# arpitbansal297/Cold-Diffusion-Models

Measured on NVIDIA H100. Metric: training-step images/sec (CelebA-128 deblur UNet, config 3), higher is better.
Workload: dtype tf32

## Files before the change

### cold_diffusion_models_b200/csrc/wgrad_tc.cu

```cuda
#include "tc_common.cuh"

namespace {

constexpr int kMmaWarps = 8;
constexpr int kThreads = 32 * (kMmaWarps + 1);
constexpr int kMaxTaps = 8;
constexpr int kMaxGroups = 4;
constexpr int kMaxAccCols = 256;

struct WgParams {
  int B, Hg, Wg;
  int CW, R, KR;
  int chunks_x, chunks_y, total_chunks, chunks_per_split, splits;
  int Cout, Cin;
  int tiles_co, tiles_ci;
  int ngroups;
  int ntaps[kMaxGroups];
  int nloads[kMaxGroups];
  int tap_index[kMaxGroups][kMaxTaps];
  int tap_load[kMaxGroups][kMaxTaps];
  int tap_shift[kMaxGroups][kMaxTaps];
  int load_dy[kMaxGroups][kMaxTaps], load_dx[kMaxGroups][kMaxTaps];
  int halo;
  int sy, sx;
  int oys, oxs, oy0, ox0;
  int per_batch, chunks_per_img, splits_per_img;
  long long dw_batch_stride;
  float* dw;
  float* db;
};

__device__ __forceinline__ float lds_sw(const uint8_t* base, int row, int c) {
  return cd_round_tf32(*reinterpret_cast<const float*>(base + row * 128 + ((((c >> 2) ^ row) & 7) << 4) + (c & 3) * 4));
}
__device__ __forceinline__ void mma_tf32_16x8x8(float (&d)[4], const float (&a)[4], const float (&b)[2]) {
  asm volatile("mma.sync.aligned.m16n8k8.row.col.f32.tf32.tf32.f32 {%0, %1, %2, %3}, {%4, %5, %6, %7}, {%8, %9}, {%0, %1, %2, %3};"
               : "+f"(d[0]), "+f"(d[1]), "+f"(d[2]), "+f"(d[3])
               : "r"(__float_as_uint(a[0])), "r"(__float_as_uint(a[1])), "r"(__float_as_uint(a[2])), "r"(__float_as_uint(a[3])),
                 "r"(__float_as_uint(b[0])), "r"(__float_as_uint(b[1])));
}
__device__ __forceinline__ void red_add_v2(float* addr, float a, float b) {
  asm volatile("red.global.add.v2.f32 [%0], {%1, %2};" :: "l"(addr), "f"(a), "f"(b) : "memory");
}

template <int BN, int NT, bool BIAS>
__global__ void __launch_bounds__(kThreads, 1)
wgrad_tc_kernel(const __grid_constant__ CUtensorMap mapDY, const __grid_constant__ CUtensorMap mapX,
                const WgParams p, int stages, int a_bytes, int b_bytes, int b_tx_bytes) {
  constexpr int NCH = BN / 32;
  constexpr int NJ = BN / 16;
  static_assert(NT * BN <= kMaxAccCols, "accumulators of one CTA");
  extern __shared__ uint8_t smem_raw[];
  const uint32_t raw_addr = smem_u32(smem_raw);
  uint8_t* smem = smem_raw + ((1024u - (raw_addr & 1023u)) & 1023u);
  const int g = blockIdx.z;
  const int nl = p.nloads[g];
  const int stage_bytes = a_bytes + nl * b_bytes;
  uint64_t* bars = reinterpret_cast<uint64_t*>(smem + stages * stage_bytes);
  uint64_t* full_bar = bars;
  uint64_t* empty_bar = bars + stages;
  const int warp = threadIdx.x >> 5, lane = threadIdx.x & 31;

  if (threadIdx.x == 0) {
    for (int i = 0; i < stages; ++i) { mbar_init(&full_bar[i], 1); mbar_init(&empty_bar[i], kMmaWarps); }
    asm volatile("fence.mbarrier_init.release.cluster;" ::: "memory");
  }
  __syncthreads();

  const int tile = blockIdx.x;
  const int co0 = (tile % p.tiles_co) * 128, ci0 = (tile / p.tiles_co) * BN;
  const int split = blockIdx.y;
  int c_beg = split * p.chunks_per_split;
  int c_end = c_beg + p.chunks_per_split; if (c_end > p.total_chunks) c_end = p.total_chunks;
  long long dw_off = 0;
  if (p.per_batch) {
    const int n = split / p.splits_per_img, sp = split % p.splits_per_img;
    c_beg = n * p.chunks_per_img + sp * p.chunks_per_split;
    c_end = c_beg + p.chunks_per_split;
    if (c_end > (n + 1) * p.chunks_per_img) c_end = (n + 1) * p.chunks_per_img;
    dw_off = n * p.dw_batch_stride;
  }
  const int nchunks = c_end > c_beg ? c_end - c_beg : 0;
// ... 63 lines not shown
#pragma unroll
      for (int t = 0; t < NT; ++t) {
        const uint8_t* sBt = sB + tap_load[t] * b_bytes;
#pragma unroll
        for (int j = 0; j < NJ; ++j) {
          const int cl = wn * (BN / 2) + j * 8 + gq;
          const uint8_t* sBc = sBt + (cl >> 5) * (b_bytes / NCH);
          const float b[2] = {lds_sw(sBc, r0 + tap_shift[t], cl & 31), lds_sw(sBc, r1 + tap_shift[t], cl & 31)};
          mma_tf32_16x8x8(acc[t][0][j], a[0], b);
          mma_tf32_16x8x8(acc[t][1][j], a[1], b);
        }
      }
    }
    __syncwarp();
    if (lane == 0) mbar_arrive(&empty_bar[stage]);
  }
  if (nchunks == 0) return;
#pragma unroll
  for (int t = 0; t < NT; ++t) {
    if (t >= p.ntaps[g]) break;
#pragma unroll
    for (int i = 0; i < 2; ++i) {
#pragma unroll
      for (int h = 0; h < 2; ++h) {
        const int co = co0 + wm * 32 + i * 16 + gq + h * 8;
        if (co >= p.Cout) continue;
        float* wrow = p.dw + dw_off + (static_cast<long long>(p.tap_index[g][t]) * p.Cout + co) * p.Cin;
#pragma unroll
        for (int j = 0; j < NJ; ++j) {
          const int ci = ci0 + wn * (BN / 2) + j * 8 + tq * 2;
          if (ci < p.Cin) red_add_v2(wrow + ci, acc[t][i][j][2 * h], acc[t][i][j][2 * h + 1]);
        }
      }
    }
  }
  if (BIAS && bias_cta) {
#pragma unroll
    for (int i = 0; i < 2; ++i)
#pragma unroll
      for (int h = 0; h < 2; ++h) {
        float v = bsum[i][h];
        v += __shfl_xor_sync(0xffffffffu, v, 1);
        v += __shfl_xor_sync(0xffffffffu, v, 2);
        const int co = co0 + wm * 32 + i * 16 + gq + h * 8;
        if (tq == 0 && co < p.Cout) atomicAdd(p.db + co, v);
      }
  }
}

constexpr int kWmThreads = 512;
constexpr int kWmKR = 64;
constexpr int kWmRegsLow = 40, kWmRegsHigh = 216;

template <int CW> struct WmGeom {
  static constexpr int R = kWmKR / CW, RL = CW + 8;
  static constexpr int kXBox = RL * (R + 2) * 128;
  static constexpr int kXBytes = 2 * kXBox;
  static_assert(kXBox % 1024 == 0, "X boxes keep 1024-byte alignment");
};
template <int BN> struct WmTiles {
  static constexpr int kRawBox = kWmKR * 128;
  static constexpr int kRawBytes = (BN / 32) * kRawBox;
  static constexpr int kBBytes = BN * kWmKR * 4;
};

template <int BN, int NTW, int CW>
__device__ __forceinline__ void wm_consume(const WgParams& p, const uint8_t* smem, int stages, int stage_bytes, uint64_t* afull,
                                           uint64_t* aempty, uint64_t* bfull, uint64_t* bempty, int nchunks, int g, int tbeg,
                                           int co0, int ci0) {
  using G = WmGeom<CW>;
  using T = WmTiles<BN>;
  const int lane = threadIdx.x & 31, w = (threadIdx.x & 127) >> 5, gq = lane >> 2, tq = lane & 3;
  int off[NTW][4];
  const int c = 16 * (w & 1) + gq;
#pragma unroll
  for (int t = 0; t < NTW; ++t) {
#pragma unroll
    for (int h = 0; h < 2; ++h) {
      const int row = p.tap_shift[g][tbeg + t] + 2 * tq + h;
      const int o = (w >> 1) * G::kXBox + row * 128 + ((((c >> 2) ^ row) & 7) << 4) + (c & 3) * 4;
      off[t][2 * h] = o;
      off[t][2 * h + 1] = o ^ 32;
    }
  }
  float acc[NTW][BN / 2];
  uint32_t fr[2][NTW][4];
  auto load_frags = [&](uint32_t (&f)[NTW][4], const uint8_t* xs, int ks) {
    const int kofs = (((ks * 8) / CW) * G::RL + (ks * 8) % CW) * 128;
#pragma unroll
    for (int t = 0; t < NTW; ++t)
#pragma unroll
      for (int e = 0; e < 4; ++e) f[t][e] = __float_as_uint(cd_round_tf32(*reinterpret_cast<const float*>(xs + off[t][e] + kofs)));
  };
  if (nchunks == 0) return;
  mbar_wait(&afull[0], 0);
  load_frags(fr[0], smem, 0);
  for (int it = 0; it < nchunks; ++it) {
    const uint32_t s = it % stages, ph = (it / stages) & 1u;
    mbar_wait(&bfull[s], ph);
    const uint8_t* xs = smem + s * stage_bytes;
    const uint32_t bs = smem_u32(xs + G::kXBytes + T::kRawBytes);
#pragma unroll
    for (int ks = 0; ks < kWmKR / 8; ++ks) {
      wgmma_fence();
      const uint64_t db = make_kmajor_sw128_desc(bs + (ks >> 2) * (BN * 128)) + uint64_t((ks & 3) * 2);
#pragma unroll
      for (int t = 0; t < NTW; ++t) wgmma_tf32_rs<BN>(acc[t], fr[ks & 1][t], db, (it | ks) != 0 ? 1u : 0u);
      wgmma_commit();
      if (ks + 1 < kWmKR / 8) {
        load_frags(fr[(ks + 1) & 1], xs, ks + 1);
      } else if (it + 1 < nchunks) {
        const uint32_t s1 = (it + 1) % stages, ph1 = ((it + 1) / stages) & 1u;
        mbar_wait(&afull[s1], ph1);
        load_frags(fr[0], smem + s1 * stage_bytes, 0);
      }
      wgmma_wait<0>();
    }
    __syncwarp();
    if (lane == 0) { mbar_arrive(&aempty[s]); mbar_arrive(&bempty[s]); }
  }
#pragma unroll
  for (int t = 0; t < NTW; ++t) {
    float* wt = p.dw + static_cast<long long>(p.tap_index[g][tbeg + t]) * p.Cout * p.Cin + ci0 + 16 * w + gq;
#pragma unroll
    for (int j = 0; j < BN / 8; ++j)
#pragma unroll
      for (int e = 0; e < 4; ++e) {
        const int co = co0 + 8 * j + 2 * tq + (e & 1);
        if (co < p.Cout) atomicAdd(wt + static_cast<long long>(co) * p.Cin + (e >> 1) * 8, acc[t][4 * j + e]);
      }
  }
}

template <int BN, int NT, int CW>
__global__ void __launch_bounds__(kWmThreads, 1)
wgrad_wgmma_kernel(const __grid_constant__ CUtensorMap mapDY, const __grid_constant__ CUtensorMap mapX, const __grid_constant__ WgParams p,
                   int stages) {
  using G = WmGeom<CW>;
  using T = WmTiles<BN>;
  constexpr int kStage = G::kXBytes + T::kRawBytes + T::kBBytes;
  extern __shared__ uint8_t smem_raw[];
  const uint32_t raw_addr = smem_u32(smem_raw);
  uint8_t* smem = smem_raw + ((1024u - (raw_addr & 1023u)) & 1023u);
  uint64_t* bars = reinterpret_cast<uint64_t*>(smem + stages * kStage);
  uint64_t* afull = bars;
  uint64_t* aempty = bars + stages;
  uint64_t* rfull = bars + 2 * stages;
  uint64_t* rempty = bars + 3 * stages;
  uint64_t* bfull = bars + 4 * stages;
  uint64_t* bempty = bars + 5 * stages;
  const int warp = threadIdx.x >> 5, lane = threadIdx.x & 31, wg = threadIdx.x >> 7;
  const int g = blockIdx.z, nt = p.ntaps[g];
  const int ncons = nt > NT ? 2 : 1;
  if (threadIdx.x == 0) {
    for (int i = 0; i < stages; ++i) {
      mbar_init(&afull[i], 1); mbar_init(&aempty[i], 4 * ncons);
      mbar_init(&rfull[i], 1); mbar_init(&rempty[i], 4);
      mbar_init(&bfull[i], 4); mbar_init(&bempty[i], 4 * ncons);
    }
    asm volatile("fence.mbarrier_init.release.cluster;" ::: "memory");
  }
  __syncthreads();

  const int tile = blockIdx.x;
  const int co0 = (tile % p.tiles_co) * BN, ci0 = (tile / p.tiles_co) * 64;
  const int c_beg = blockIdx.y * p.chunks_per_split;
  int c_end = c_beg + p.chunks_per_split; if (c_end > p.total_chunks) c_end = p.total_chunks;
  const int nchunks = c_end > c_beg ? c_end - c_beg : 0;

  if (wg == 0) {
    asm volatile("setmaxnreg.dec.sync.aligned.u32 %0;" :: "n"(kWmRegsLow));
    if (warp != 0) return;
    for (int it = 0; it < nchunks; ++it) {
      const int ch = c_beg + it;
      const int gx0 = (ch % p.chunks_x) * CW, gy0 = ((ch / p.chunks_x) % p.chunks_y) * G::R, n = ch / (p.chunks_x * p.chunks_y);
      const uint32_t s = it % stages, ph = (it / stages) & 1u;
      const uint32_t sx = smem_u32(smem + s * kStage);
      mbar_wait(&rempty[s], ph ^ 1u);
      if (elect_one()) {
        mbar_expect_tx(&rfull[s], T::kRawBytes);
#pragma unroll
        for (int b = 0; b < BN / 32; ++b)
          tma_load_4d(sx + G::kXBytes + b * T::kRawBox, &mapDY, &rfull[s], co0 + 32 * b, gx0, gy0, n);
      }
      __syncwarp();
      mbar_wait(&aempty[s], ph ^ 1u);
      if (elect_one()) {
        mbar_expect_tx(&afull[s], G::kXBytes);
        tma_load_4d(sx, &mapX, &afull[s], ci0, gx0 - 1, gy0 - 1, n);
        tma_load_4d(sx + G::kXBox, &mapX, &afull[s], ci0 + 32, gx0 - 1, gy0 - 1, n);
      }
      __syncwarp();
    }
    return;
  }
  if (wg == 1) {
    asm volatile("setmaxnreg.dec.sync.aligned.u32 %0;" :: "n"(kWmRegsLow));
    const int w4 = warp & 3;
    for (int it = 0; it < nchunks; ++it) {
      const uint32_t s = it % stages, ph = (it / stages) & 1u;
      mbar_wait(&rfull[s], ph);
      mbar_wait(&bempty[s], ph ^ 1u);
      const uint8_t* raw = smem + s * kStage + G::kXBytes;
      uint8_t* bt = smem + s * kStage + G::kXBytes + T::kRawBytes;
#pragma unroll 4
      for (int u = w4; u < (BN / 32) * (kWmKR / 4); u += 4) {
        const int b = u % (BN / 32), kq = u / (BN / 32);
        const int co = 32 * b + lane;
        const uint8_t* src = raw + b * T::kRawBox + (lane & 3) * 4;
        float v[4];
#pragma unroll
        for (int j = 0; j < 4; ++j) {
          const int px = 8 * (kq >> 1) + (kq & 1) + 2 * j;
          v[j] = cd_round_tf32(*reinterpret_cast<const float*>(src + px * 128 + ((((lane >> 2) ^ px) & 7) << 4)));
        }
        *reinterpret_cast<float4*>(bt + (kq >> 3) * (BN * 128) + co * 128 + (((kq ^ co) & 7) << 4)) = make_float4(v[0], v[1], v[2], v[3]);
      }
      asm volatile("fence.proxy.async.shared::cta;" ::: "memory");
      __syncwarp();
      if (lane == 0) { mbar_arrive(&rempty[s]); mbar_arrive(&bfull[s]); }
    }
    return;
  }
  const int tbeg = (wg - 2) * NT;
  const int ntw = nt - tbeg < NT ? nt - tbeg : NT;
  if (ntw <= 0) return;
  asm volatile("setmaxnreg.inc.sync.aligned.u32 %0;" :: "n"(kWmRegsHigh));
  if constexpr (NT == 4) {
    if (ntw == 4) wm_consume<BN, 4, CW>(p, smem, stages, kStage, afull, aempty, bfull, bempty, nchunks, g, tbeg, co0, ci0);
    else if (ntw == 3) wm_consume<BN, 3, CW>(p, smem, stages, kStage, afull, aempty, bfull, bempty, nchunks, g, tbeg, co0, ci0);
    else if (ntw == 2) wm_consume<BN, 2, CW>(p, smem, stages, kStage, afull, aempty, bfull, bempty, nchunks, g, tbeg, co0, ci0);
    else wm_consume<BN, 1, CW>(p, smem, stages, kStage, afull, aempty, bfull, bempty, nchunks, g, tbeg, co0, ci0);
  } else {
    if (ntw == 2) wm_consume<BN, 2, CW>(p, smem, stages, kStage, afull, aempty, bfull, bempty, nchunks, g, tbeg, co0, ci0);
    else wm_consume<BN, 1, CW>(p, smem, stages, kStage, afull, aempty, bfull, bempty, nchunks, g, tbeg, co0, ci0);
  }
}

int g_wg_mode = 1;
int g_sms = 0;

template <int BN, int NT>
int launch_wg(bool bias, dim3 grid, size_t smem, cudaStream_t st, const CUtensorMap& mapDY, const CUtensorMap& mapX,
              const WgParams& p, int stages, int a_bytes, int b_bytes, int b_tx) {
  if (bias) {
    CD_CUDA(cudaFuncSetAttribute(wgrad_tc_kernel<BN, NT, true>, cudaFuncAttributeMaxDynamicSharedMemorySize, (int)smem));
    wgrad_tc_kernel<BN, NT, true><<<grid, kThreads, smem, st>>>(mapDY, mapX, p, stages, a_bytes, b_bytes, b_tx);
  } else {
    CD_CUDA(cudaFuncSetAttribute(wgrad_tc_kernel<BN, NT, false>, cudaFuncAttributeMaxDynamicSharedMemorySize, (int)smem));
    wgrad_tc_kernel<BN, NT, false><<<grid, kThreads, smem, st>>>(mapDY, mapX, p, stages, a_bytes, b_bytes, b_tx);
  }
  CD_LAUNCH_CHECK();
  return 0;
}

}

extern "C" int cd_wgrad_tc_set_mode(int mode) { g_wg_mode = mode; return 0; }

static int g_wg_bias_fusion = 0;
extern "C" int cd_wgrad_tc_set_bias_fusion(int enable) { g_wg_bias_fusion = enable; return 0; }

static int g_split_policy = 3;
static int g_split_over_clk = 12000;
extern "C" int cd_wgrad_tc_set_split(int policy, int over_clk) { g_split_policy = policy; if (over_clk > 0) g_split_over_clk = over_clk; return 0; }

static int choose_splits(int tg, int total_chunks, int max_splits, int sms, double chunk_clk) {
  if (max_splits < 1) max_splits = 1;
  int s;
  if (g_split_policy == 0) s = cd_cdiv(2 * sms, tg);
  else if (g_split_policy == 1) s = sms / tg;
  else if (g_split_policy == 2) s = 2 * sms / tg;
  else {
    double best = 1e30; s = 1;
    for (int c = 1; c <= max_splits && c * tg <= 4 * sms + tg; ++c) {
      const int cps = cd_cdiv(total_chunks, c);
      const int real = cd_cdiv(total_chunks, cps);
      const double cost = double(cd_cdiv(static_cast<long long>(tg) * real, sms)) * (cps * chunk_clk + g_split_over_clk);
      if (cost < best) { best = cost; s = c; }
    }
  }
  if (s > max_splits) s = max_splits;
  if (s < 1) s = 1;
  return s;
}

template <int BN, int NT, int CW>
static int launch_wm(dim3 grid, cudaStream_t st, const CUtensorMap& mapDY, const CUtensorMap& mapX, const WgParams& p) {
  constexpr int kStage = WmGeom<CW>::kXBytes + WmTiles<BN>::kRawBytes + WmTiles<BN>::kBBytes;
  int stages = (224 * 1024) / kStage; if (stages > 5) stages = 5;
  static_assert((224 * 1024) / kStage >= 2, "two stages of the wgmma weight-gradient kernel fit shared memory");
  const size_t smem = size_t(stages) * kStage + 1024 + 256;
  auto kern = wgrad_wgmma_kernel<BN, NT, CW>;
  static bool attr_done = false;
  if (!attr_done) {
    CD_CUDA(cudaFuncSetAttribute(kern, cudaFuncAttributeMaxDynamicSharedMemorySize, (int)smem));
    attr_done = true;
  }
  kern<<<grid, kWmThreads, smem, st>>>(mapDY, mapX, p, stages);
  CD_LAUNCH_CHECK();
  return 0;
}

static int wgrad_wgmma(const CdConvDesc* d, const float* dout, int dout_ld, float* dw, EncodeTiledFn enc, cudaStream_t st) {
  const CdConvSrc& c = d->s[0];
  if (c.w_per_batch || d->sy != 1 || d->sx != 1 || d->oys != 1 || d->oxs != 1 || d->oy0 != 0 || d->ox0 != 0) return 1;
  if (c.H != d->Hg || c.W != d->Wg || d->Ho != d->Hg || d->Wo != d->Wg) return 1;
  if (c.C % 64 != 0 || d->Cout % 64 != 0 || c.ntaps < 2 || c.ntaps > 9) return 1;
  for (int t = 0; t < c.ntaps; ++t) if (c.dy[t] < -1 || c.dy[t] > 1 || c.dx[t] < -1 || c.dx[t] > 1) return 1;
  const int CW = d->Wg >= 16 ? 16 : 8, R = kWmKR / CW;
  if (d->Hg < R) return 1;
  const int BN = d->Cout % 128 == 0 ? 128 : 64;
  const int NT = BN == 128 ? 2 : 4;
  WgParams p{};
  p.B = d->B; p.Hg = d->Hg; p.Wg = d->Wg; p.Cout = d->Cout; p.Cin = c.C;
  p.sy = 1; p.sx = 1; p.oys = 1; p.oxs = 1;
  p.dw = dw;
  p.CW = CW; p.R = R; p.KR = kWmKR;
  p.ngroups = cd_cdiv(c.ntaps, 2 * NT);
  for (int gk = 0; gk < p.ngroups; ++gk) {
    const int t0 = gk * 2 * NT, n = c.ntaps - t0 < 2 * NT ? c.ntaps - t0 : 2 * NT;
    p.ntaps[gk] = n;
    for (int k = 0; k < n; ++k) {
      p.tap_index[gk][k] = t0 + k;
      p.tap_shift[gk][k] = (c.dy[t0 + k] + 1) * (CW + 8) + c.dx[t0 + k] + 1;
    }
  }
  p.chunks_x = d->Wg / CW; p.chunks_y = d->Hg / R;
  p.total_chunks = d->B * p.chunks_x * p.chunks_y;
  p.tiles_co = d->Cout / BN; p.tiles_ci = c.C / 64;
  const int tiles = p.tiles_co * p.tiles_ci;
  const int max_taps = p.ntaps[0];
  const double chunk_clk = double(max_taps) * (kWmKR / 8) * (BN / 2);
  const int splits = choose_splits(tiles * p.ngroups, p.total_chunks, cd_cdiv(p.total_chunks, 8), g_sms, chunk_clk);
  p.chunks_per_split = cd_cdiv(p.total_chunks, splits);
  p.splits = cd_cdiv(p.total_chunks, p.chunks_per_split);

  CUtensorMap mapDY, mapX;
  const CUtensorMapDataType dt = CU_TENSOR_MAP_DATA_TYPE_FLOAT32;
  {
    cuuint64_t dims[4] = {(cuuint64_t)d->Cout, (cuuint64_t)d->Wo, (cuuint64_t)d->Ho, (cuuint64_t)d->B};
    cuuint64_t strides[3] = {(cuuint64_t)dout_ld * 4, (cuuint64_t)dout_ld * 4 * d->Wo, (cuuint64_t)dout_ld * 4 * d->Wo * d->Ho};
    cuuint32_t box[4] = {32, (cuuint32_t)CW, (cuuint32_t)R, 1};
    cuuint32_t estr[4] = {1, 1, 1, 1};
    CUresult r = enc(&mapDY, dt, 4, const_cast<float*>(dout), dims, strides, box, estr, CU_TENSOR_MAP_INTERLEAVE_NONE,
                     CU_TENSOR_MAP_SWIZZLE_128B, CU_TENSOR_MAP_L2_PROMOTION_L2_128B, CU_TENSOR_MAP_FLOAT_OOB_FILL_NONE);
    CD_REQUIRE(r == CUDA_SUCCESS, "cuTensorMapEncodeTiled(wgmma dY) failed: %d", (int)r);
  }
  {
    cuuint64_t dims[4] = {(cuuint64_t)c.C, (cuuint64_t)c.W, (cuuint64_t)c.H, (cuuint64_t)d->B};
    cuuint64_t strides[3] = {(cuuint64_t)c.ld * 4, (cuuint64_t)c.ld * 4 * c.W, (cuuint64_t)c.ld * 4 * c.W * c.H};
    cuuint32_t box[4] = {32, (cuuint32_t)(CW + 8), (cuuint32_t)(R + 2), 1};
    cuuint32_t estr[4] = {1, 1, 1, 1};
    CUresult r = enc(&mapX, dt, 4, const_cast<float*>(c.src), dims, strides, box, estr, CU_TENSOR_MAP_INTERLEAVE_NONE,
                     CU_TENSOR_MAP_SWIZZLE_128B, CU_TENSOR_MAP_L2_PROMOTION_L2_128B, CU_TENSOR_MAP_FLOAT_OOB_FILL_NONE);
    CD_REQUIRE(r == CUDA_SUCCESS, "cuTensorMapEncodeTiled(wgmma X) failed: %d", (int)r);
  }
  const dim3 grid(tiles, p.splits, p.ngroups);
  if (BN == 128) return CW == 16 ? launch_wm<128, 2, 16>(grid, st, mapDY, mapX, p) : launch_wm<128, 2, 8>(grid, st, mapDY, mapX, p);
  return CW == 16 ? launch_wm<64, 4, 16>(grid, st, mapDY, mapX, p) : launch_wm<64, 4, 8>(grid, st, mapDY, mapX, p);
}

int cd_conv_wgrad_tc(const CdConvDesc* d, const float* dout, int dout_ld, float* dw, float* db, int* bias_done, cudaStream_t st) {
  if (bias_done) *bias_done = 0;
  const CdConvSrc& c = d->s[0];
  if (c.C % 32 != 0 || d->Cout % 32 != 0 || c.ld % 4 != 0 || dout_ld % 4 != 0) return 1;
  if (!is_pow2(d->Wg) || d->Wg < 8 || !is_pow2(d->Hg)) return 1;
  if ((reinterpret_cast<uintptr_t>(c.src) & 15) || (reinterpret_cast<uintptr_t>(dout) & 15) || (reinterpret_cast<uintptr_t>(dw) & 15)) return 1;
  EncodeTiledFn enc = get_encode();
  CD_REQUIRE(enc != nullptr, "cuTensorMapEncodeTiled entry point unavailable");
  if (!g_sms) { int dev = 0; CD_CUDA(cudaGetDevice(&dev)); CD_CUDA(cudaDeviceGetAttribute(&g_sms, cudaDevAttrMultiProcessorCount, dev)); }
  if (g_wg_mode != 0 && g_wg_mode != 8 && !(g_wg_bias_fusion && db != nullptr)) {
    const int r = wgrad_wgmma(d, dout, dout_ld, dw, enc, st);
    if (r <= 0) return r;
  }

  WgParams p{};
  p.B = d->B; p.Hg = d->Hg; p.Wg = d->Wg; p.Cout = d->Cout; p.Cin = c.C;
  p.sy = d->sy; p.sx = d->sx; p.oys = d->oys; p.oxs = d->oxs; p.oy0 = d->oy0; p.ox0 = d->ox0;
  p.dw = dw;
  int BN = c.C >= 128 ? 128 : 64;
  const bool is3x3 = (c.ntaps == 9 && d->sy == 1 && d->sx == 1);
  bool shape3 = is3x3;
  if (is3x3) for (int t = 0; t < 9; ++t) if (c.dy[t] != t / 3 - 1 || c.dx[t] != t % 3 - 1) shape3 = false;
  const bool halo = shape3 && g_wg_mode != 0;
  p.halo = halo ? 2 : 0;
  if (halo) {
    p.ngroups = 3;
    for (int gk = 0; gk < 3; ++gk) {
      p.ntaps[gk] = 3; p.nloads[gk] = 1; p.load_dy[gk][0] = gk - 1; p.load_dx[gk][0] = -1;
      for (int k = 0; k < 3; ++k) { p.tap_index[gk][k] = gk * 3 + k; p.tap_load[gk][k] = 0; p.tap_shift[gk][k] = k; }
    }
  } else {
    const int per = c.ntaps <= 4 ? c.ntaps : (c.ntaps == 9 ? 3 : 4);
    if (c.ntaps % per != 0 || c.ntaps / per > kMaxGroups) return 1;
    p.ngroups = c.ntaps / per;
    for (int gk = 0; gk < p.ngroups; ++gk) {
      p.ntaps[gk] = per; p.nloads[gk] = per;
      for (int k = 0; k < per; ++k) {
        const int t = gk * per + k;
        p.tap_index[gk][k] = t; p.tap_load[gk][k] = k; p.tap_shift[gk][k] = 0;
        p.load_dy[gk][k] = c.dy[t]; p.load_dx[gk][k] = c.dx[t];
      }
    }
  }
  const int max_taps = p.ntaps[0], max_loads = p.nloads[0];
  if (max_taps * BN > kMaxAccCols) BN = 64;
  if (max_taps * BN > kMaxAccCols) return 1;
  int KR = (max_loads <= 1) ? 64 : 32;
  if (static_cast<long long>(d->Hg) * d->Wg < KR) KR = d->Hg * d->Wg;
  if (KR < 8) return 1;
  p.CW = d->Wg < KR ? d->Wg : KR;
  p.R = KR / p.CW;
// ... 70 lines not shown
```

### cold_diffusion_models_b200/engine_bwd.py

```python
import ctypes as C
import torch

from . import ops
from .ops import View, CONV_TC, CONV_SIMT, ACT_NONE, ACT_GELU_BWD
from ._lib import call, ptr, stream
from .engine import T1, T3, T4, T3D, TPAR, _tc_ok

NULL = C.c_void_p(0)


def flat_offsets(named_numels):
    table, off = {}, 0
    for n, k in named_numels:
        table[n] = (off, k)
        off += (k + 31) // 32 * 32
    return table, off


def allreduce_mean_(flat_grad, world):
    if world > 1:
        torch.distributed.all_reduce(flat_grad)
    return 1.0 / world


# ... 175 lines not shown
        self._wgrad(hv, T3, bs.dmid, grid, View(dpre), G[pn + '.net.1.weight'], G[pn + '.net.1.bias'], key=pn + '.w1', real_c=edge_c)
        ld_in = sv.get('ld_h', hv.ld)
        dhn = self.buf('g.hn.%dx%dx%d' % (H, W, ld_in), (B, H, W, ld_in))
        d = ops.make_conv_desc([(View(dpre), T3D, P[pn + '.w1T'], False)], View(dhn, 0, bs.din), grid, Cout=bs.din)
        self._conv(d, True)
        if bs.has_norm:
            dh = self.buf('g.h.%dx%dx%d' % (H, W, ld_in), (B, H, W, ld_in))
            call('cd_layernorm_bwd', ptr(dhn), ld_in, ptr(hpre), ld_in, ptr(stats), ptr(m.net[0].g), C.c_int64(B * H * W),
                 bs.din, NULL, 0, ptr(dh), ld_in, ptr(G[pn + '.net.0.g']), ptr(G[pn + '.net.0.b']), stream())
        else:
            dh = dhn
        if bs.cond_off is not None:
            dslice = C.c_void_p(self._dcond.data_ptr() + 4 * bs.cond_off)
            call('cd_colsum_batched', ptr(dh), ld_in, B, C.c_int64(H * W), bs.din, dslice, self.sumC, stream())
            call('cd_colsum', dslice, self.sumC, C.c_int64(B), bs.din, ptr(G[pn + '.ds_conv.bias']), stream())
        else:
            call('cd_colsum', ptr(dh), ld_in, C.c_int64(B * H * W), bs.din, ptr(G[pn + '.ds_conv.bias']), stream())
        call('cd_dwconv7_wgrad', ptr(dh), ld_in, C.c_void_p(xv.addr()), xv.ld, B, H, W, bs.din,
             ptr(G[pn + '.ds_conv.weight']), stream())
        if not need_dx:
            return None
        if bs.has_res:
            r = self.buf('g.r.%dx%dx%d' % (H, W, ld_in), (B, H, W, ld_in))
            d = ops.make_conv_desc([(dyv, T1, P[pn + '.wrT'], False)], View(r, 0, bs.din), grid, Cout=bs.din)
            self._conv(d, _tc_ok(bs.dout))
            addv = View(r, 0, bs.din)
        else:
            addv = dyv
        dx = self.buf('g.x.' + pn, (B, H, W, ld_in))
        if bs.din % 32 == 0:
            call('cd_dwconv7_fwd', ptr(dh), ld_in, B, H, W, bs.din, ptr(m.ds_conv.weight), NULL, NULL, 0, ptr(dx), ld_in, 1,
                 C.c_void_p(addv.addr()), addv.ld, stream())
        else:
            call('cd_dwconv7_ln_fwd', ptr(dh), ld_in, B, H, W, bs.din, ptr(m.ds_conv.weight), NULL, NULL, 0, NULL, NULL,
                 C.c_float(0.0), ptr(dx), ld_in, NULL, NULL, 0, 0, 1, C.c_void_p(addv.addr()), addv.ld, stream())
        return View(dx, 0, bs.din)

    def _attn_bwd(self, spec, save, dyv):
        sv = save[spec.name]
        xv, xnv, qkv, kmax, ksum, ctx, weff, stats = sv['x'], sv['xn'], sv['qkv'], sv['kmax'], sv['ksum'], sv['ctx'], sv['weff'], sv['stats']
        B, H, W = xv.B, xv.H, xv.W
        n = H * W
        dim = spec.dim
        a = spec.attn
        P, G = self._packed, self.G
        pn = spec.name + '.fn'
        grid = (B, H, W)
        tc_pb = n >= 128
        call('cd_colsum', C.c_void_p(dyv.addr()), dyv.ld, C.c_int64(B * n), dim, ptr(G[pn + '.fn.to_out.bias']), stream())
        dweff = self.buf('g.dweff', (B, dim, 128))
        dweff.zero_()
        qv = View(qkv, 0, 128)
        d = ops.make_conv_desc([(qv, T1, dweff, True)], dyv, grid, Cout=dim)
        ops.conv_wgrad(d, dyv, dweff, None, impl=self.conv_impl)
        dctxn = self.buf('g.dctxn', (B, 4, 32, 32))
        rowdot = self.buf('g.rowdot', (B, 128))
        call('cd_linattn_bwd_small', ptr(dweff), ptr(ctx), ptr(ksum), ptr(a.to_out.weight), B, dim, C.c_float(a.scale),
             ptr(G[pn + '.fn.to_out.weight']), ptr(dctxn), ptr(rowdot), stream())
        dqkv = self.buf('g.qkv.%dx%d' % (H, W), (B, H, W, 384))
        wt = self.buf('g.wefft', (B, 128, dim))
        call('cd_transpose_weff', ptr(weff), B, dim, ptr(wt), stream())
        d = ops.make_conv_desc([(dyv, T1, wt, True)], View(dqkv, 0, 128), grid, Cout=128)
        self._conv(d, tc_pb and _tc_ok(dim))
        call('cd_linattn_bwd_kv', ptr(qkv), 384, B, n, ptr(kmax), ptr(ksum), ptr(dctxn), ptr(rowdot), ptr(dqkv), 384, stream())
        self._wgrad(xnv, T1, 384, grid, View(dqkv), G[pn + '.fn.to_qkv.weight'], None, key=spec.name + '.wqkv')
        dxn = self.buf('g.xn.%dx%dx%d' % (H, W, dim), (B, H, W, dim))
        d = ops.make_conv_desc([(View(dqkv), T1, P[spec.name + '.wqkvT'], False)], View(dxn), grid, Cout=dim)
        self._conv(d, True)
        dx = self.buf('g.x.' + spec.name, (B, H, W, dim))
        call('cd_layernorm_bwd', ptr(dxn), dim, C.c_void_p(xv.addr()), xv.ld, ptr(stats), ptr(spec.norm.g), C.c_int64(B * n),
             dim, C.c_void_p(dyv.addr()), dyv.ld, ptr(dx), dim, ptr(G[pn + '.norm.g']), ptr(G[pn + '.norm.b']), stream())
        return View(dx)

    def backward(self, save, dout):
        unet = self.unet
        shape, gen = save.get('_gen', (None, None))
        if shape is not None and self._gen_by_shape.get(shape) != gen:
            raise RuntimeError("Unet backward: another forward with input shape %r ran on this network after the forward being "
                               "differentiated; the engine keeps one set of saved activations per input shape -- call "
                               "backward() before the next forward (e.g. accumulate micro-batches one at a time)" % (shape,))
        self._setup_grads()
        self.prepare_weights_bwd()
        P, G = self._packed, self.G
        dout = dout.contiguous().float()
        B = dout.shape[0]
        self._unpack_batch = self._repack_batch('unpack', 'unpack') if self.profile_wgrads is None else None
        if self._unpack_batch is None or self._dwp_clean is None or getattr(self, '_dwp_pending', False):
            self._dwp_clean = {}
        self._dwp_pending = self._unpack_batch is not None
        self._dwp_seen = set()
        self._dcond = self.buf('g.dcond', (B, max(self.sumC, 1)))
        self._dcond.zero_()
        nd, nu = len(self.levels_down), len(self.levels_up)
        fx = save['final']['x']
        h, w = fx.H, fx.W
        dfo = self.buf('g.final', (B, h, w, fx.ld))
        od = self.final_proj.weight.shape[0]
        call('cd_conv1x1_to_nchw_bwd', ptr(dout), ptr(fx.t), fx.ld, B, h, w, fx.C, ptr(self.final_proj.weight), od,
             ptr(dfo), fx.ld, ptr(G['final_conv.1.weight']), ptr(G['final_conv.1.bias']), stream())
        d = self._block_bwd(self.final_block, save, View(dfo))
        dskip = {}
        for k in reversed(range(nu)):
            b0, b1, at, up = self.levels_up[k]
            if up is not None:
                sv = save['ups.%d.3' % k]
                xv = sv['x']
                c = xv.C
# ... 92 lines not shown
```

Baseline: 589.1.

## Extend wgmma weight-gradient kernel to 1x1, stride-2, parity, Cin=32 and per-batch convs

```diff
diff --git a/cold_diffusion_models_b200/csrc/wgrad_tc.cu b/cold_diffusion_models_b200/csrc/wgrad_tc.cu
--- a/cold_diffusion_models_b200/csrc/wgrad_tc.cu
+++ b/cold_diffusion_models_b200/csrc/wgrad_tc.cu
@@ -28,6 +28,8 @@
   long long dw_batch_stride;
   float* dw;
   float* db;
+  int wm_nbox[kMaxGroups], ci_tile;
+  int wm_box[kMaxGroups][kMaxTaps][2], wm_shift[kMaxGroups][kMaxTaps][2], wm_tap[kMaxGroups][kMaxTaps][2];
 };
 
 __device__ __forceinline__ float lds_sw(const uint8_t* base, int row, int c) {
@@ -197,10 +199,9 @@
 constexpr int kWmKR = 64;
 constexpr int kWmRegsLow = 40, kWmRegsHigh = 216;
 
-template <int CW> struct WmGeom {
-  static constexpr int R = kWmKR / CW, RL = CW + 8;
-  static constexpr int kXBox = RL * (R + 2) * 128;
-  static constexpr int kXBytes = 2 * kXBox;
+template <int CW, bool HALO> struct WmGeom {
+  static constexpr int R = kWmKR / CW, RL = HALO ? CW + 8 : CW;
+  static constexpr int kXBox = RL * (R + (HALO ? 2 : 0)) * 128;
   static_assert(kXBox % 1024 == 0, "X boxes keep 1024-byte alignment");
 };
 template <int BN> struct WmTiles {
@@ -208,24 +209,29 @@
   static constexpr int kRawBytes = (BN / 32) * kRawBox;
   static constexpr int kBBytes = BN * kWmKR * 4;
 };
-
-template <int BN, int NTW, int CW>
-__device__ __forceinline__ void wm_consume(const WgParams& p, const uint8_t* smem, int stages, int stage_bytes, uint64_t* afull,
-                                           uint64_t* aempty, uint64_t* bfull, uint64_t* bempty, int nchunks, int g, int tbeg,
-                                           int co0, int ci0) {
-  using G = WmGeom<CW>;
+constexpr int wm_slots_1x1(int BN) { return BN == 128 ? 3 : 4; }
+template <int BN, int CW, bool HALO> struct WmStage {
+  static constexpr int kXBytes = (HALO ? 2 : 2 * wm_slots_1x1(BN)) * WmGeom<CW, HALO>::kXBox;
+  static constexpr int kBytes = WmTiles<BN>::kRawBytes + WmTiles<BN>::kBBytes + kXBytes;
+  static_assert((224 * 1024) / kBytes >= 2, "two stages of the wgmma weight-gradient kernel fit shared memory");
+};
+
+template <int BN, int NTW, int CW, bool HALO>
+__device__ __forceinline__ void wm_consume(const WgParams& p, const uint8_t* smem, int stages, int stage_bytes,
+                                           uint64_t* afull, uint64_t* aempty, uint64_t* bfull, uint64_t* bempty, int nchunks, int g,
+                                           int tbeg, int co0, int ci0) {
+  using G = WmGeom<CW, HALO>;
   using T = WmTiles<BN>;
   const int lane = threadIdx.x & 31, w = (threadIdx.x & 127) >> 5, gq = lane >> 2, tq = lane & 3;
-  int off[NTW][4];
+  int off[NTW][2];
   const int c = 16 * (w & 1) + gq;
 #pragma unroll
   for (int t = 0; t < NTW; ++t) {
 #pragma unroll
     for (int h = 0; h < 2; ++h) {
-      const int row = p.tap_shift[g][tbeg + t] + 2 * tq + h;
-      const int o = (w >> 1) * G::kXBox + row * 128 + ((((c >> 2) ^ row) & 7) << 4) + (c & 3) * 4;
-      off[t][2 * h] = o;
-      off[t][2 * h + 1] = o ^ 32;
+      const int row = ((NTW <= 2 && p.Cin == 32) ? p.wm_shift[g][tbeg + t][w >> 1] : p.wm_shift[g][tbeg + t][0]) + 2 * tq + h;
+      const int box = (NTW <= 2 && p.Cin == 32) ? 0 : (HALO ? 0 : 2 * (tbeg + t)) + (w >> 1);
+      off[t][h] = box * G::kXBox + row * 128 + ((((c >> 2) ^ row) & 7) << 4) + (c & 3) * 4;
     }
   }
   float acc[NTW][BN / 2];
@@ -235,16 +241,17 @@
 #pragma unroll
     for (int t = 0; t < NTW; ++t)
 #pragma unroll
-      for (int e = 0; e < 4; ++e) f[t][e] = __float_as_uint(cd_round_tf32(*reinterpret_cast<const float*>(xs + off[t][e] + kofs)));
+      for (int e = 0; e < 4; ++e)
+        f[t][e] = __float_as_uint(cd_round_tf32(*reinterpret_cast<const float*>(xs + (off[t][e >> 1] ^ ((e & 1) * 32)) + kofs)));
   };
   if (nchunks == 0) return;
   mbar_wait(&afull[0], 0);
-  load_frags(fr[0], smem, 0);
+  load_frags(fr[0], smem + T::kRawBytes + T::kBBytes, 0);
   for (int it = 0; it < nchunks; ++it) {
     const uint32_t s = it % stages, ph = (it / stages) & 1u;
     mbar_wait(&bfull[s], ph);
-    const uint8_t* xs = smem + s * stage_bytes;
-    const uint32_t bs = smem_u32(xs + G::kXBytes + T::kRawBytes);
+    const uint8_t* xs = smem + s * stage_bytes + T::kRawBytes + T::kBBytes;
+    const uint32_t bs = smem_u32(smem + s * stage_bytes + T::kRawBytes);
 #pragma unroll
     for (int ks = 0; ks < kWmKR / 8; ++ks) {
       wgmma_fence();
@@ -257,16 +264,21 @@
       } else if (it + 1 < nchunks) {
         const uint32_t s1 = (it + 1) % stages, ph1 = ((it + 1) / stages) & 1u;
         mbar_wait(&afull[s1], ph1);
-        load_frags(fr[0], smem + s1 * stage_bytes, 0);
+        load_frags(fr[0], smem + s1 * stage_bytes + T::kRawBytes + T::kBBytes, 0);
       }
       wgmma_wait<0>();
     }
     __syncwarp();
     if (lane == 0) { mbar_arrive(&aempty[s]); mbar_arrive(&bempty[s]); }
   }
+  asm volatile("" ::: "memory");
+  const long long dw_off = p.per_batch ? (blockIdx.y / p.splits_per_img) * p.dw_batch_stride : 0;
 #pragma unroll
   for (int t = 0; t < NTW; ++t) {
-    float* wt = p.dw + static_cast<long long>(p.tap_index[g][tbeg + t]) * p.Cout * p.Cin + ci0 + 16 * w + gq;
+    const int tap = p.wm_tap[g][tbeg + t][w >> 1];
+    if (tap < 0) continue;
+    float* wt = p.dw + dw_off + static_cast<long long>(tap) * p.Cout * p.Cin + ci0 + 32 * p.wm_box[g][tbeg + t][w >> 1] +
+                16 * (w & 1) + gq;
 #pragma unroll
     for (int j = 0; j < BN / 8; ++j)
 #pragma unroll
@@ -277,13 +289,13 @@
   }
 }
 
-template <int BN, int NT, int CW>
+template <int BN, int NT, int CW, bool HALO>
 __global__ void __launch_bounds__(kWmThreads, 1)
 wgrad_wgmma_kernel(const __grid_constant__ CUtensorMap mapDY, const __grid_constant__ CUtensorMap mapX, const __grid_constant__ WgParams p,
                    int stages) {
-  using G = WmGeom<CW>;
+  using G = WmGeom<CW, HALO>;
   using T = WmTiles<BN>;
-  constexpr int kStage = G::kXBytes + T::kRawBytes + T::kBBytes;
+  constexpr int kStage = WmStage<BN, CW, HALO>::kBytes;
   extern __shared__ uint8_t smem_raw[];
   const uint32_t raw_addr = smem_u32(smem_raw);
   uint8_t* smem = smem_raw + ((1024u - (raw_addr & 1023u)) & 1023u);
@@ -296,7 +308,7 @@
   uint64_t* bempty = bars + 5 * stages;
   const int warp = threadIdx.x >> 5, lane = threadIdx.x & 31, wg = threadIdx.x >> 7;
   const int g = blockIdx.z, nt = p.ntaps[g];
-  const int ncons = nt > NT ? 2 : 1;
+  const int ncons = nt > 1 ? 2 : 1;
   if (threadIdx.x == 0) {
     for (int i = 0; i < stages; ++i) {
       mbar_init(&afull[i], 1); mbar_init(&aempty[i], 4 * ncons);
@@ -308,9 +320,15 @@
   __syncthreads();
 
   const int tile = blockIdx.x;
-  const int co0 = (tile % p.tiles_co) * BN, ci0 = (tile / p.tiles_co) * 64;
-  const int c_beg = blockIdx.y * p.chunks_per_split;
+  const int co0 = (tile % p.tiles_co) * BN, ci0 = (tile / p.tiles_co) * p.ci_tile;
+  int c_beg = blockIdx.y * p.chunks_per_split;
   int c_end = c_beg + p.chunks_per_split; if (c_end > p.total_chunks) c_end = p.total_chunks;
+  if (p.per_batch) {
+    const int n = blockIdx.y / p.splits_per_img, sp = blockIdx.y % p.splits_per_img;
+    c_beg = n * p.chunks_per_img + sp * p.chunks_per_split;
+    c_end = c_beg + p.chunks_per_split;
+    if (c_end > (n + 1) * p.chunks_per_img) c_end = (n + 1) * p.chunks_per_img;
+  }
   const int nchunks = c_end > c_beg ? c_end - c_beg : 0;
 
   if (wg == 0) {
@@ -326,14 +344,15 @@
         mbar_expect_tx(&rfull[s], T::kRawBytes);
 #pragma unroll
         for (int b = 0; b < BN / 32; ++b)
-          tma_load_4d(sx + G::kXBytes + b * T::kRawBox, &mapDY, &rfull[s], co0 + 32 * b, gx0, gy0, n);
+          tma_load_4d(sx + b * T::kRawBox, &mapDY, &rfull[s], co0 + 32 * b, gx0, gy0, n);
       }
       __syncwarp();
       mbar_wait(&aempty[s], ph ^ 1u);
       if (elect_one()) {
-        mbar_expect_tx(&afull[s], G::kXBytes);
-        tma_load_4d(sx, &mapX, &afull[s], ci0, gx0 - 1, gy0 - 1, n);
-        tma_load_4d(sx + G::kXBox, &mapX, &afull[s], ci0 + 32, gx0 - 1, gy0 - 1, n);
+        const int nb = p.wm_nbox[g], h = HALO ? 1 : 0;
+        mbar_expect_tx(&afull[s], nb * G::kXBox);
+        for (int b = 0; b < nb; ++b)
+          tma_load_4d(sx + T::kRawBytes + T::kBBytes + b * G::kXBox, &mapX, &afull[s], ci0 + 32 * b, gx0 - h, gy0 - h, n);
       }
       __syncwarp();
     }
@@ -346,8 +365,8 @@
       const uint32_t s = it % stages, ph = (it / stages) & 1u;
       mbar_wait(&rfull[s], ph);
       mbar_wait(&bempty[s], ph ^ 1u);
-      const uint8_t* raw = smem + s * kStage + G::kXBytes;
-      uint8_t* bt = smem + s * kStage + G::kXBytes + T::kRawBytes;
+      const uint8_t* raw = smem + s * kStage;
+      uint8_t* bt = smem + s * kStage + T::kRawBytes;
 #pragma unroll 4
       for (int u = w4; u < (BN / 32) * (kWmKR / 4); u += 4) {
         const int b = u % (BN / 32), kq = u / (BN / 32);
@@ -367,19 +386,22 @@
     }
     return;
   }
-  const int tbeg = (wg - 2) * NT;
-  const int ntw = nt - tbeg < NT ? nt - tbeg : NT;
+  const int half = (nt + 1) / 2;
+  const int tbeg = (wg - 2) * half;
+  const int ntw = wg == 2 ? half : nt - half;
   if (ntw <= 0) return;
   asm volatile("setmaxnreg.inc.sync.aligned.u32 %0;" :: "n"(kWmRegsHigh));
-  if constexpr (NT == 4) {
-    if (ntw == 4) wm_consume<BN, 4, CW>(p, smem, stages, kStage, afull, aempty, bfull, bempty, nchunks, g, tbeg, co0, ci0);
-    else if (ntw == 3) wm_consume<BN, 3, CW>(p, smem, stages, kStage, afull, aempty, bfull, bempty, nchunks, g, tbeg, co0, ci0);
-    else if (ntw == 2) wm_consume<BN, 2, CW>(p, smem, stages, kStage, afull, aempty, bfull, bempty, nchunks, g, tbeg, co0, ci0);
-    else wm_consume<BN, 1, CW>(p, smem, stages, kStage, afull, aempty, bfull, bempty, nchunks, g, tbeg, co0, ci0);
+#define WM_CONSUME(n) wm_consume<BN, n, CW, HALO>(p, smem, stages, kStage, afull, aempty, bfull, bempty, nchunks, g, tbeg, co0, ci0)
+  if constexpr (NT == 4 && HALO) {
+    if (ntw == 4) WM_CONSUME(4);
+    else if (ntw == 3) WM_CONSUME(3);
+    else if (ntw == 2) WM_CONSUME(2);
+    else WM_CONSUME(1);
   } else {
-    if (ntw == 2) wm_consume<BN, 2, CW>(p, smem, stages, kStage, afull, aempty, bfull, bempty, nchunks, g, tbeg, co0, ci0);
-    else wm_consume<BN, 1, CW>(p, smem, stages, kStage, afull, aempty, bfull, bempty, nchunks, g, tbeg, co0, ci0);
-  }
+    if (ntw == 2) WM_CONSUME(2);
+    else WM_CONSUME(1);
+  }
+#undef WM_CONSUME
 }
 
 int g_wg_mode = 1;
@@ -430,16 +452,17 @@
   return s;
 }
 
-template <int BN, int NT, int CW>
+constexpr int kWmSmem = 224 * 1024 + 1024 + 256;
+
+template <int BN, int NT, int CW, bool HALO>
 static int launch_wm(dim3 grid, cudaStream_t st, const CUtensorMap& mapDY, const CUtensorMap& mapX, const WgParams& p) {
-  constexpr int kStage = WmGeom<CW>::kXBytes + WmTiles<BN>::kRawBytes + WmTiles<BN>::kBBytes;
+  constexpr int kStage = WmStage<BN, CW, HALO>::kBytes;
   int stages = (224 * 1024) / kStage; if (stages > 5) stages = 5;
-  static_assert((224 * 1024) / kStage >= 2, "two stages of the wgmma weight-gradient kernel fit shared memory");
   const size_t smem = size_t(stages) * kStage + 1024 + 256;
-  auto kern = wgrad_wgmma_kernel<BN, NT, CW>;
+  auto kern = wgrad_wgmma_kernel<BN, NT, CW, HALO>;
   static bool attr_done = false;
   if (!attr_done) {
-    CD_CUDA(cudaFuncSetAttribute(kern, cudaFuncAttributeMaxDynamicSharedMemorySize, (int)smem));
+    CD_CUDA(cudaFuncSetAttribute(kern, cudaFuncAttributeMaxDynamicSharedMemorySize, kWmSmem));
     attr_done = true;
   }
   kern<<<grid, kWmThreads, smem, st>>>(mapDY, mapX, p, stages);
@@ -447,63 +470,127 @@
   return 0;
 }
 
+static int encode_nhwc(EncodeTiledFn enc, CUtensorMap* m, const float* base, int ld, int C, int W0, int H0, int B, int sy, int sx,
+                        int ey, int ex, int W, int H, int bw, int bh, const char* what) {
+  cuuint64_t dims[4] = {(cuuint64_t)C, (cuuint64_t)W, (cuuint64_t)H, (cuuint64_t)B};
+  cuuint64_t strides[3] = {(cuuint64_t)ld * 4 * sx, (cuuint64_t)ld * 4 * W0 * sy, (cuuint64_t)ld * 4 * W0 * H0};
+  cuuint32_t box[4] = {32, (cuuint32_t)bw, (cuuint32_t)bh, 1};
+  cuuint32_t estr[4] = {1, 1, 1, 1};
+  float* p = const_cast<float*>(base) + (static_cast<long long>(ey) * W0 + ex) * ld;
+  CUresult r = enc(m, CU_TENSOR_MAP_DATA_TYPE_FLOAT32, 4, p, dims, strides, box, estr, CU_TENSOR_MAP_INTERLEAVE_NONE,
+                   CU_TENSOR_MAP_SWIZZLE_128B, CU_TENSOR_MAP_L2_PROMOTION_L2_128B, CU_TENSOR_MAP_FLOAT_OOB_FILL_NONE);
+  CD_REQUIRE(r == CUDA_SUCCESS, "cuTensorMapEncodeTiled(%s) failed: %d", what, (int)r);
+  return 0;
+}
+
+struct WmClass { int ey, ex, n, tap[16], sy[16], sx[16]; };
+
+static int wm_plan(const CdConvDesc* d, const WmClass& k, int BN, int CW, WgParams& p, bool& halo) {
+  const int Cin = d->s[0].C, NT = BN == 128 ? 2 : 4;
+  halo = !(k.n == 1 && k.sy[0] == 0 && k.sx[0] == 0);
+  p.tiles_co = d->Cout / BN;
+  int sb[16][2], ss[16][2], st[16][2], ns = 0, nbox = 2;
+  auto shift = [&](int i) { return halo ? (k.sy[i] + 1) * (CW + 8) + k.sx[i] + 1 : 0; };
+  if (Cin == 32) {
+    if (halo && BN != 128) return 1;
+    nbox = 1;
+    for (int i = 0; i < k.n; i += 2, ++ns)
+      for (int h = 0; h < 2; ++h) {
+        const bool on = i + h < k.n;
+        sb[ns][h] = 0; ss[ns][h] = on ? shift(i + h) : 0; st[ns][h] = on ? k.tap[i + h] : -1;
+      }
+  } else if (!halo) {
+    ns = wm_slots_1x1(BN);
+    while ((Cin / 64) % ns != 0) --ns;
+    nbox = 2 * ns;
+    for (int t = 0; t < ns; ++t)
+      for (int h = 0; h < 2; ++h) { sb[t][h] = 2 * t + h; ss[t][h] = 0; st[t][h] = k.tap[0]; }
+  } else {
+    for (int i = 0; i < k.n; ++i, ++ns)
+      for (int h = 0; h < 2; ++h) { sb[ns][h] = h; ss[ns][h] = shift(i); st[ns][h] = k.tap[i]; }
+  }
+  p.ci_tile = Cin == 32 ? 32 : 32 * nbox;
+  p.tiles_ci = Cin == 32 ? 1 : Cin / p.ci_tile;
+  p.ngroups = cd_cdiv(ns, 2 * NT);
+  if (p.ngroups > kMaxGroups) return 1;
+  for (int g = 0; g < p.ngroups; ++g) {
+    const int s0 = g * 2 * NT, n = ns - s0 < 2 * NT ? ns - s0 : 2 * NT;
+    p.ntaps[g] = n;
+    p.wm_nbox[g] = nbox;
+    for (int t = 0; t < n; ++t)
+      for (int h = 0; h < 2; ++h) { p.wm_box[g][t][h] = sb[s0 + t][h]; p.wm_shift[g][t][h] = ss[s0 + t][h]; p.wm_tap[g][t][h] = st[s0 + t][h]; }
+  }
+  return 0;
+}
+
 static int wgrad_wgmma(const CdConvDesc* d, const float* dout, int dout_ld, float* dw, EncodeTiledFn enc, cudaStream_t st) {
   const CdConvSrc& c = d->s[0];
-  if (c.w_per_batch || d->sy != 1 || d->sx != 1 || d->oys != 1 || d->oxs != 1 || d->oy0 != 0 || d->ox0 != 0) return 1;
-  if (c.H != d->Hg || c.W != d->Wg || d->Ho != d->Hg || d->Wo != d->Wg) return 1;
-  if (c.C % 64 != 0 || d->Cout % 64 != 0 || c.ntaps < 2 || c.ntaps > 9) return 1;
-  for (int t = 0; t < c.ntaps; ++t) if (c.dy[t] < -1 || c.dy[t] > 1 || c.dx[t] < -1 || c.dx[t] > 1) return 1;
+  if ((c.C % 64 != 0 && c.C != 32) || d->Cout % 64 != 0 || c.ntaps < 1) return 1;
+  const bool dense_out = d->oys == 1 && d->oxs == 1 && d->oy0 == 0 && d->ox0 == 0 && d->Ho == d->Hg && d->Wo == d->Wg;
+  const bool parity_out = d->oys == 2 && d->oxs == 2 && (d->oy0 & ~1) == 0 && (d->ox0 & ~1) == 0 && d->Ho == 2 * d->Hg &&
+                          d->Wo == 2 * d->Wg;
+  const bool s1 = d->sy == 1 && d->sx == 1 && c.H == d->Hg && c.W == d->Wg && (dense_out || parity_out);
+  const bool s2 = d->sy == 2 && d->sx == 2 && c.H == 2 * d->Hg && c.W == 2 * d->Wg && dense_out;
+  if (!s1 && !s2) return 1;
   const int CW = d->Wg >= 16 ? 16 : 8, R = kWmKR / CW;
   if (d->Hg < R) return 1;
   const int BN = d->Cout % 128 == 0 ? 128 : 64;
-  const int NT = BN == 128 ? 2 : 4;
-  WgParams p{};
-  p.B = d->B; p.Hg = d->Hg; p.Wg = d->Wg; p.Cout = d->Cout; p.Cin = c.C;
-  p.sy = 1; p.sx = 1; p.oys = 1; p.oxs = 1;
-  p.dw = dw;
-  p.CW = CW; p.R = R; p.KR = kWmKR;
-  p.ngroups = cd_cdiv(c.ntaps, 2 * NT);
-  for (int gk = 0; gk < p.ngroups; ++gk) {
-    const int t0 = gk * 2 * NT, n = c.ntaps - t0 < 2 * NT ? c.ntaps - t0 : 2 * NT;
-    p.ntaps[gk] = n;
-    for (int k = 0; k < n; ++k) {
-      p.tap_index[gk][k] = t0 + k;
-      p.tap_shift[gk][k] = (c.dy[t0 + k] + 1) * (CW + 8) + c.dx[t0 + k] + 1;
-    }
-  }
-  p.chunks_x = d->Wg / CW; p.chunks_y = d->Hg / R;
-  p.total_chunks = d->B * p.chunks_x * p.chunks_y;
-  p.tiles_co = d->Cout / BN; p.tiles_ci = c.C / 64;
-  const int tiles = p.tiles_co * p.tiles_ci;
-  const int max_taps = p.ntaps[0];
-  const double chunk_clk = double(max_taps) * (kWmKR / 8) * (BN / 2);
-  const int splits = choose_splits(tiles * p.ngroups, p.total_chunks, cd_cdiv(p.total_chunks, 8), g_sms, chunk_clk);
-  p.chunks_per_split = cd_cdiv(p.total_chunks, splits);
-  p.splits = cd_cdiv(p.total_chunks, p.chunks_per_split);
-
-  CUtensorMap mapDY, mapX;
-  const CUtensorMapDataType dt = CU_TENSOR_MAP_DATA_TYPE_FLOAT32;
-  {
-    cuuint64_t dims[4] = {(cuuint64_t)d->Cout, (cuuint64_t)d->Wo, (cuuint64_t)d->Ho, (cuuint64_t)d->B};
-    cuuint64_t strides[3] = {(cuuint64_t)dout_ld * 4, (cuuint64_t)dout_ld * 4 * d->Wo, (cuuint64_t)dout_ld * 4 * d->Wo * d->Ho};
-    cuuint32_t box[4] = {32, (cuuint32_t)CW, (cuuint32_t)R, 1};
-    cuuint32_t estr[4] = {1, 1, 1, 1};
-    CUresult r = enc(&mapDY, dt, 4, const_cast<float*>(dout), dims, strides, box, estr, CU_TENSOR_MAP_INTERLEAVE_NONE,
-                     CU_TENSOR_MAP_SWIZZLE_128B, CU_TENSOR_MAP_L2_PROMOTION_L2_128B, CU_TENSOR_MAP_FLOAT_OOB_FILL_NONE);
-    CD_REQUIRE(r == CUDA_SUCCESS, "cuTensorMapEncodeTiled(wgmma dY) failed: %d", (int)r);
-  }
-  {
-    cuuint64_t dims[4] = {(cuuint64_t)c.C, (cuuint64_t)c.W, (cuuint64_t)c.H, (cuuint64_t)d->B};
-    cuuint64_t strides[3] = {(cuuint64_t)c.ld * 4, (cuuint64_t)c.ld * 4 * c.W, (cuuint64_t)c.ld * 4 * c.W * c.H};
-    cuuint32_t box[4] = {32, (cuuint32_t)(CW + 8), (cuuint32_t)(R + 2), 1};
-    cuuint32_t estr[4] = {1, 1, 1, 1};
-    CUresult r = enc(&mapX, dt, 4, const_cast<float*>(c.src), dims, strides, box, estr, CU_TENSOR_MAP_INTERLEAVE_NONE,
-                     CU_TENSOR_MAP_SWIZZLE_128B, CU_TENSOR_MAP_L2_PROMOTION_L2_128B, CU_TENSOR_MAP_FLOAT_OOB_FILL_NONE);
-    CD_REQUIRE(r == CUDA_SUCCESS, "cuTensorMapEncodeTiled(wgmma X) failed: %d", (int)r);
-  }
-  const dim3 grid(tiles, p.splits, p.ngroups);
-  if (BN == 128) return CW == 16 ? launch_wm<128, 2, 16>(grid, st, mapDY, mapX, p) : launch_wm<128, 2, 8>(grid, st, mapDY, mapX, p);
-  return CW == 16 ? launch_wm<64, 4, 16>(grid, st, mapDY, mapX, p) : launch_wm<64, 4, 8>(grid, st, mapDY, mapX, p);
+  WmClass cls[4];
+  int ncls = 0;
+  for (int e = 0; e < (s2 ? 4 : 1); ++e) {
+    WmClass& k = cls[ncls];
+    k.ey = e >> 1; k.ex = e & 1; k.n = 0;
+    for (int t = 0; t < c.ntaps; ++t) {
+      if (s2 && ((c.dy[t] & 1) != k.ey || (c.dx[t] & 1) != k.ex)) continue;
+      const int sy = s2 ? (c.dy[t] - k.ey) / 2 : c.dy[t], sx = s2 ? (c.dx[t] - k.ex) / 2 : c.dx[t];
+      if (sy < -1 || sy > 1 || sx < -1 || sx > 1) return 1;
+      k.tap[k.n] = t; k.sy[k.n] = sy; k.sx[k.n] = sx; ++k.n;
+    }
+    if (k.n > 0) ++ncls;
+  }
+  WgParams ps[4];
+  bool halo[4];
+  for (int i = 0; i < ncls; ++i) {
+    ps[i] = WgParams{};
+    if (wm_plan(d, cls[i], BN, CW, ps[i], halo[i])) return 1;
+  }
+  CUtensorMap mapDY;
+  if (encode_nhwc(enc, &mapDY, dout, dout_ld, d->Cout, d->Wo, d->Ho, d->B, d->oys, d->oxs, d->oy0, d->ox0, d->Wg, d->Hg, CW, R, "wgmma dY")) return -1;
+  for (int i = 0; i < ncls; ++i) {
+    WgParams& p = ps[i];
+    p.B = d->B; p.Hg = d->Hg; p.Wg = d->Wg; p.Cout = d->Cout; p.Cin = c.C;
+    p.dw = dw;
+    p.CW = CW; p.R = R; p.KR = kWmKR;
+    p.chunks_x = d->Wg / CW; p.chunks_y = d->Hg / R;
+    p.total_chunks = d->B * p.chunks_x * p.chunks_y;
+    const int tiles = p.tiles_co * p.tiles_ci;
+    const double chunk_clk = double(p.ntaps[0]) * (kWmKR / 8) * (BN / 2);
+    if (c.w_per_batch) {
+      p.per_batch = 1;
+      p.chunks_per_img = p.chunks_x * p.chunks_y;
+      const int spi = choose_splits(tiles * p.ngroups * d->B, p.chunks_per_img, p.chunks_per_img, g_sms, chunk_clk);
+      p.chunks_per_split = cd_cdiv(p.chunks_per_img, spi);
+      p.splits_per_img = cd_cdiv(p.chunks_per_img, p.chunks_per_split);
+      p.splits = p.splits_per_img * d->B;
+      p.dw_batch_stride = static_cast<long long>(c.ntaps) * d->Cout * c.C;
+    } else {
+      const int splits = choose_splits(tiles * p.ngroups, p.total_chunks, cd_cdiv(p.total_chunks, 8), g_sms, chunk_clk);
+      p.chunks_per_split = cd_cdiv(p.total_chunks, splits);
+      p.splits = cd_cdiv(p.total_chunks, p.chunks_per_split);
+    }
+    CUtensorMap mapX;
+    const int bw = halo[i] ? CW + 8 : CW, bh = halo[i] ? R + 2 : R;
+    if (encode_nhwc(enc, &mapX, c.src, c.ld, c.C, c.W, c.H, d->B, d->sy, d->sx, cls[i].ey, cls[i].ex, d->Wg, d->Hg, bw, bh, "wgmma X")) return -1;
+    const dim3 grid(tiles, p.splits, p.ngroups);
+#define WM_LAUNCH(bn, nt, cw) (halo[i] ? launch_wm<bn, nt, cw, true>(grid, st, mapDY, mapX, p) \
+                                       : launch_wm<bn, nt, cw, false>(grid, st, mapDY, mapX, p))
+    int rc;
+    if (BN == 128) rc = CW == 16 ? WM_LAUNCH(128, 2, 16) : WM_LAUNCH(128, 2, 8);
+    else rc = CW == 16 ? WM_LAUNCH(64, 4, 16) : WM_LAUNCH(64, 4, 8);
+#undef WM_LAUNCH
+    if (rc) return rc;
+  }
+  return 0;
 }
 
 int cd_conv_wgrad_tc(const CdConvDesc* d, const float* dout, int dout_ld, float* dw, float* db, int* bias_done, cudaStream_t st) {
diff --git a/cold_diffusion_models_b200/engine_bwd.py b/cold_diffusion_models_b200/engine_bwd.py
--- a/cold_diffusion_models_b200/engine_bwd.py
+++ b/cold_diffusion_models_b200/engine_bwd.py
@@ -251,7 +251,14 @@
         dweff.zero_()
         qv = View(qkv, 0, 128)
         d = ops.make_conv_desc([(qv, T1, dweff, True)], dyv, grid, Cout=dim)
-        ops.conv_wgrad(d, dyv, dweff, None, impl=self.conv_impl)
+        if self.profile_wgrads is not None:
+            e0, e1 = torch.cuda.Event(enable_timing=True), torch.cuda.Event(enable_timing=True)
+            e0.record()
+            ops.conv_wgrad(d, dyv, dweff, None, impl=self.conv_impl)
+            e1.record()
+            self.profile_wgrads.append((e0, e1, (B, H, W, dim, 128, 1, 'batch')))
+        else:
+            ops.conv_wgrad(d, dyv, dweff, None, impl=self.conv_impl)
         dctxn = self.buf('g.dctxn', (B, 4, 32, 32))
         rowdot = self.buf('g.rowdot', (B, 128))
         call('cd_linattn_bwd_small', ptr(dweff), ptr(ctx), ptr(ksum), ptr(a.to_out.weight), B, dim, C.c_float(a.scale),
```

Result: faster. 617.1 (median of 6 runs) (+4.8%).
